# QuentinFuxa/WhisperLiveKit

Hardware: AMD Instinct MI355X
Metric: audio seconds transcribed per second (1/RTF), Whisper-base EN simul_whisper AlignAtt, 0.5 s chunks (higher is better)
Workload: dtype f32; 1 GPU; base.en simul_whisper, 1 stream(s) over 1 GPU(s) (1 per GPU), 30 s 16 kHz speech-like stream, 0.5 s chunks, beam 1, frame_threshold 25, seeded random weights, synthetic vocabulary; model=base.en, streams_total=1

## Files before the change

include/wlk_hip.h:

```cpp
#ifndef WLK_HIP_H
#define WLK_HIP_H

#include <stdint.h>

#ifdef __cplusplus
extern "C" {
#endif

#define WLK_OK 0
#define WLK_ERR_ARG (-1)
#define WLK_ERR_HIP (-2)
#define WLK_ERR_STATE (-3)
#define WLK_ERR_CAPACITY (-4)

typedef struct wlk_model wlk_model;
typedef struct wlk_session wlk_session;

typedef struct wlk_dims {
    int32_t n_mels, n_audio_ctx, n_audio_state, n_audio_head, n_audio_layer;
    int32_t n_vocab, n_text_ctx, n_text_state, n_text_head, n_text_layer;
} wlk_dims;

const char* wlk_last_error(void);
int wlk_abi_version(void);
// ... 159 lines not shown
int wlk_diag_env_refresh(void);
int wlk_diag_linear(const float* a, int64_t lda, int64_t a_floats, const float* w, const float* bias,
                    const float* r, int64_t ldr, int m, int n, int k, int flags, float scale, int scale_cols,
                    int force_gemv, float* c);
typedef struct wlk_nllb_dims {
    int32_t vocab, d_model, heads, ffn, enc_layers, dec_layers;
    int32_t max_src, max_tgt;
    int32_t pad_id;
    int32_t n_positions;
    float embed_scale;
} wlk_nllb_dims;
typedef struct wlk_nllb wlk_nllb;
typedef struct wlk_nllb_session wlk_nllb_session;
int wlk_nllb_arena_floats(const wlk_nllb_dims* dims, uint64_t* n_floats);
int wlk_nllb_tensor_lookup(const wlk_nllb_dims* dims, const char* packed_name, uint64_t* offset_floats, uint64_t* numel);
int wlk_nllb_tensor_name(const wlk_nllb_dims* dims, int index, const char** name);
int wlk_nllb_create(const wlk_nllb_dims* dims, int device, wlk_nllb** out);
int wlk_nllb_upload(wlk_nllb* m, const char* packed_name, const float* host, uint64_t numel);
int wlk_nllb_finalize(wlk_nllb* m);
int wlk_nllb_destroy(wlk_nllb* m);
int wlk_nllb_session_create(wlk_nllb* m, int rows, wlk_nllb_session** out);
int wlk_nllb_session_destroy(wlk_nllb_session* s);
int wlk_nllb_encode(wlk_nllb_session* s, const int64_t* src_ids, int32_t n);
int wlk_nllb_decode(wlk_nllb_session* s, const int64_t* tokens, int32_t n_rows, int32_t n_tok, int32_t first);
int wlk_nllb_step(wlk_nllb_session* s, const int64_t* tokens, int32_t n_rows, int32_t k, float* logprobs, int32_t* ids);
int wlk_nllb_kv_reorder(wlk_nllb_session* s, const int32_t* source_rows, int32_t n_rows);
int wlk_nllb_topk(wlk_nllb_session* s, int32_t k, float* logprobs, int32_t* ids);
int wlk_nllb_export(wlk_nllb_session* s, const char* what, float* host, uint64_t capacity, uint64_t* n_written);
int wlk_nllb_sync(wlk_nllb_session* s);

int wlk_dtw(int device, const float* x, int32_t n_rows, int32_t n_cols, int8_t* trace);
int wlk_log_mel(wlk_session* s, const float* pcm, int64_t n_samples, int32_t padding, float* mel, uint64_t capacity_floats,
                int32_t* n_frames);
int wlk_encode_mel(wlk_session* s, const float* mel, int32_t n_frames);
int wlk_find_alignment(wlk_session* s, const int64_t* tokens, int32_t n_tokens, int32_t n_sot, int32_t eot,
                       int32_t num_frames, float qk_scale, float* cost, int8_t* trace, float* token_probs);

int wlk_diag_linear_time(int m, int n, int k, int flags, int force_gemv, int reps, float* us_per_launch);
int wlk_diag_linear_ln(const float* a, const float* w, const float* bias, const float* gamma, const float* beta,
                       int m, int n, int k, int force_gemv, float* c);
int wlk_diag_layernorm(const float* x, const float* gamma, const float* beta, int rows, int d, float* y);
int wlk_diag_prefill_stack(wlk_session** sessions, const int64_t* tokens, const int32_t* n_tok, const int32_t* sot_index, int32_t n,
                           int32_t* taken);
int wlk_engine_prefill_stats(wlk_model* m, uint64_t* batches, uint64_t* sessions);
int wlk_diag_encoder_attention_time(int t, int d, int n_head, int k_splits, int reps, float* us_per_launch);
int wlk_diag_encoder_attention(const float* qkv, int t, int d, int n_head, float* out);
int wlk_diag_wave_ops(const float* in64, float* out640, float* ref640);
int wlk_diag_linear_x3(const float* a, const float* w, const float* bias, int m, int n, int k, int flags, float scale,
                       int scale_cols, float* c);
int wlk_diag_linear_x3_time(int m, int n, int k, int flags, int reps, float* us_per_launch);
int wlk_diag_layernorm_x3(const float* x, const float* gamma, const float* beta, int rows, int d, float* y);
int wlk_diag_encoder_attention_x3(const float* qkv, int t, int d, int n_head, float* out);
int wlk_diag_encoder_attention_x3_time(int t, int d, int n_head, int reps, float* us_per_launch);
int wlk_diag_qkv_x3_attention(const float* x, const float* w, const float* bias, int t, int d, int n_head, float scale,
                              float* out_epilogue, float* out_packed);

#ifdef __cplusplus
}
#endif
#endif
```

whisperlivekit_amd/_lib.py:

```python
from __future__ import annotations

import ctypes as C
import os
import threading
from typing import Optional


_LIB_NAME = "libwlk_hip.so"
_lock = threading.Lock()
_lib: Optional[C.CDLL] = None


class WlkError(RuntimeError):
    """Raised for every non-zero status of the C ABI (message from wlk_last_error())."""


class Dims(C.Structure):
    _fields_ = [(n, C.c_int32) for n in (
        "n_mels", "n_audio_ctx", "n_audio_state", "n_audio_head", "n_audio_layer",
        "n_vocab", "n_text_ctx", "n_text_state", "n_text_head", "n_text_layer")]


class SfDims(C.Structure):
    _fields_ = [(n, C.c_int32) for n in (
# ... 113 lines not shown
        "wlk_sf_finalize": (cint, [p]),
        "wlk_sf_step": (cint, [p, p, cint, p, cint, p, cint, C.POINTER(cint), p, cint]),
        "wlk_sf_step_pcm": (cint, [p, p, p, cint, cint, p, cint, p, cint, C.POINTER(cint), p, cint, p, cint, C.POINTER(cint), p, cint]),
        "wlk_sf_stats": (cint, [p, C.POINTER(u64), C.POINTER(u64), C.POINTER(u64)]),
        "wlk_sf_export": (cint, [p, C.c_char_p, p, u64, C.POINTER(u64)]),
        "wlk_sf_destroy": (cint, [p]),
        "wlk_nllb_arena_floats": (cint, [C.POINTER(NllbDims), C.POINTER(u64)]),
        "wlk_nllb_tensor_lookup": (cint, [C.POINTER(NllbDims), C.c_char_p, C.POINTER(u64), C.POINTER(u64)]),
        "wlk_nllb_tensor_name": (cint, [C.POINTER(NllbDims), cint, C.POINTER(C.c_char_p)]),
        "wlk_nllb_create": (cint, [C.POINTER(NllbDims), cint, C.POINTER(p)]),
        "wlk_nllb_upload": (cint, [p, C.c_char_p, p, u64]),
        "wlk_nllb_finalize": (cint, [p]),
        "wlk_nllb_destroy": (cint, [p]),
        "wlk_nllb_session_create": (cint, [p, cint, C.POINTER(p)]),
        "wlk_nllb_session_destroy": (cint, [p]),
        "wlk_nllb_encode": (cint, [p, p, i32]),
        "wlk_nllb_decode": (cint, [p, p, i32, i32, i32]),
        "wlk_nllb_step": (cint, [p, p, i32, i32, p, p]),
        "wlk_nllb_kv_reorder": (cint, [p, p, i32]),
        "wlk_nllb_topk": (cint, [p, i32, p, p]),
        "wlk_nllb_export": (cint, [p, C.c_char_p, p, u64, C.POINTER(u64)]),
        "wlk_nllb_sync": (cint, [p]),
        "wlk_vad_weights_floats": (cint, [C.POINTER(u64)]),
        "wlk_vad_tensor_lookup": (cint, [C.c_char_p, C.POINTER(u64), C.POINTER(u64)]),
        "wlk_vad_tensor_name": (cint, [cint, C.POINTER(C.c_char_p)]),
        "wlk_vad_create": (cint, [cint, p, u64, C.POINTER(p)]),
        "wlk_vad_destroy": (cint, [p]),
        "wlk_vad_stream_create": (cint, [p, cint, C.POINTER(p)]),
        "wlk_vad_stream_reset": (cint, [p]),
        "wlk_vad_stream_run": (cint, [p, p, cint, p]),
        "wlk_vad_stream_state": (cint, [p, p, p]),
        "wlk_vad_stream_destroy": (cint, [p]),
        "wlk_diag_last_error": (C.c_char_p, []),
        "wlk_diag_linear": (cint, [p, C.c_int64, C.c_int64, p, p, p, C.c_int64, cint, cint, cint, cint, C.c_float,
                                   cint, cint, p]),
        "wlk_dtw": (cint, [cint, C.POINTER(C.c_float), C.c_int32, C.c_int32, C.POINTER(C.c_int8)]),
        "wlk_encode_mel": (cint, [C.c_void_p, C.POINTER(C.c_float), C.c_int32]),
        "wlk_log_mel": (cint, [C.c_void_p, C.POINTER(C.c_float), C.c_int64, C.c_int32, C.POINTER(C.c_float), C.c_uint64,
                               C.POINTER(C.c_int32)]),
        "wlk_find_alignment": (cint, [C.c_void_p, C.POINTER(C.c_int64), C.c_int32, C.c_int32, C.c_int32, C.c_int32, C.c_float,
                                      C.POINTER(C.c_float), C.POINTER(C.c_int8), C.POINTER(C.c_float)]),
        "wlk_diag_linear_time": (cint, [cint, cint, cint, cint, cint, cint, C.POINTER(C.c_float)]),
        "wlk_diag_linear_ln": (cint, [p, p, p, p, p, cint, cint, cint, cint, p]),
        "wlk_diag_layernorm": (cint, [p, p, p, cint, cint, p]),
        "wlk_diag_encoder_attention_time": (cint, [cint, cint, cint, cint, cint, C.POINTER(C.c_float)]),
        "wlk_diag_encoder_attention": (cint, [p, cint, cint, cint, p]),
        "wlk_diag_wave_ops": (cint, [p, p, p]),
        "wlk_diag_env_refresh": (cint, []),
        "wlk_diag_linear_x3": (cint, [p, p, p, cint, cint, cint, cint, C.c_float, cint, p]),
        "wlk_diag_linear_x3_time": (cint, [cint, cint, cint, cint, cint, C.POINTER(C.c_float)]),
        "wlk_diag_layernorm_x3": (cint, [p, p, p, cint, cint, p]),
        "wlk_diag_encoder_attention_x3": (cint, [p, cint, cint, cint, p]),
        "wlk_diag_encoder_attention_x3_time": (cint, [cint, cint, cint, cint, C.POINTER(C.c_float)]),
        "wlk_diag_qkv_x3_attention": (cint, [p, p, p, cint, cint, cint, C.c_float, p, p]),
    }
    for name, (res, args) in sig.items():
        try:
            fn = getattr(lib, name)
        except AttributeError:
            if "WLK_HIP_LIB" in os.environ and name.startswith("wlk_diag_"):
                continue
            raise
        fn.restype = res
        fn.argtypes = args


EXPORTED_SYMBOLS = (
    "wlk_last_error", "wlk_abi_version", "wlk_device_count", "wlk_arena_floats", "wlk_tensor_lookup",
    "wlk_tensor_name", "wlk_model_create", "wlk_model_arena", "wlk_model_upload",
    "wlk_model_set_alignment_heads", "wlk_model_finalize", "wlk_model_destroy", "wlk_session_create",
    "wlk_session_destroy", "wlk_session_set_debug", "wlk_audio_append", "wlk_audio_append_pcm16", "wlk_audio_append_zeros",
    "wlk_audio_drop_front", "wlk_audio_clear", "wlk_audio_len", "wlk_encode", "wlk_decode",
    "wlk_no_speech_prob", "wlk_rules_set", "wlk_pick_greedy", "wlk_select", "wlk_kv_reorder", "wlk_sync", "wlk_decode_until_stop", "wlk_engine_attach", "wlk_engine_detach",
    "wlk_engine_stats", "wlk_engine_encode_stats", "wlk_engine_prefill_stats", "wlk_diag_prefill_stack", "wlk_job_create",
    "wlk_job_begin_step", "wlk_job_no_speech", "wlk_job_adjustments", "wlk_job_consume", "wlk_job_result",
    "wlk_job_destroy", "wlk_export", "wlk_session_step_stats", "wlk_prof_begin",
    "wlk_prof_end", "wlk_melspec_create", "wlk_melspec_run", "wlk_melspec_destroy",
    "wlk_sf_arena_floats", "wlk_sf_tensor_lookup", "wlk_sf_tensor_name", "wlk_sf_create", "wlk_sf_upload",
    "wlk_sf_finalize", "wlk_sf_step", "wlk_sf_step_pcm", "wlk_sf_stats", "wlk_sf_export", "wlk_sf_destroy",
    "wlk_vad_weights_floats", "wlk_vad_tensor_lookup", "wlk_vad_tensor_name", "wlk_vad_create", "wlk_vad_destroy",
    "wlk_vad_stream_create", "wlk_vad_stream_reset", "wlk_vad_stream_run", "wlk_vad_stream_state",
    "wlk_vad_stream_destroy",
    "wlk_dtw", "wlk_encode_mel", "wlk_log_mel", "wlk_find_alignment",
    "wlk_nllb_arena_floats", "wlk_nllb_tensor_lookup", "wlk_nllb_tensor_name", "wlk_nllb_create", "wlk_nllb_upload",
    "wlk_nllb_finalize", "wlk_nllb_destroy", "wlk_nllb_session_create", "wlk_nllb_session_destroy", "wlk_nllb_encode",
    "wlk_nllb_decode", "wlk_nllb_step", "wlk_nllb_kv_reorder", "wlk_nllb_topk", "wlk_nllb_export", "wlk_nllb_sync",
    "wlk_diag_last_error", "wlk_diag_linear", "wlk_diag_linear_time", "wlk_diag_linear_ln", "wlk_diag_layernorm",
    "wlk_diag_encoder_attention", "wlk_diag_encoder_attention_time", "wlk_diag_wave_ops", "wlk_diag_env_refresh",
    "wlk_diag_linear_x3", "wlk_diag_linear_x3_time", "wlk_diag_layernorm_x3",
    "wlk_diag_encoder_attention_x3", "wlk_diag_encoder_attention_x3_time", "wlk_diag_qkv_x3_attention",
)


def load() -> C.CDLL:
    global _lib
    if _lib is not None:
        return _lib
    with _lock:
        if _lib is None:
            path = lib_path()
            if not os.path.exists(path):
                raise WlkError(
                    f"{path} not found: build it with `python -m whisperlivekit_amd.build` "
                    "(hipcc, gfx950). There is no CPU fallback for the HIP backend.")
            try:
                import torch
            except Exception:
                pass
            try:
                lib = C.CDLL(path, mode=C.RTLD_GLOBAL)
            except OSError as e:
                raise WlkError(f"cannot load {path}: {e}") from e
            _declare(lib)
            _lib = lib
    return _lib


def check(rc: int) -> None:
    if rc != 0:
        msg = load().wlk_last_error()
        raise WlkError(f"wlk_hip error {rc}: {msg.decode('utf-8', 'replace') if msg else '?'}")


def device_count() -> int:
    return int(load().wlk_device_count())
```

whisperlivekit_amd/csrc/attention_x3.hip:

```cpp
#include <atomic>
#include <cstdlib>
#include <type_traits>

#include "common.h"
#include "wave_ops.h"
#include "x3.h"

namespace wlk {

namespace {
typedef float af32x4 __attribute__((ext_vector_type(4)));

constexpr int AX_QT = 64, AX_KT = 32;
constexpr int AX_K_ROW = 384;
constexpr int AX_V_ROW = 192;
constexpr int AX_K_BYTES = AX_KT * AX_K_ROW;
constexpr int AX_V_BYTES = 64 * AX_V_ROW;
constexpr int AX_TILE_BYTES = AX_K_BYTES + AX_V_BYTES;
constexpr int AX_SLOT_BYTES = 2 * AX_TILE_BYTES;
constexpr int AX_NB = 3, AX_DT = AX_NB - 1;
constexpr int AX_NPW = AX_SLOT_BYTES / 1024 / 8;
constexpr size_t AX_LDS_BYTES = (size_t)AX_NB * AX_SLOT_BYTES;
constexpr int AX_PA[6] = {2, 0, 1, 1, 0, 0}, AX_PB[6] = {0, 2, 1, 0, 1, 0};

template <int N, int I = 0, typename F>
__device__ __forceinline__ void ax_static_for(F&& f) {
    if constexpr (I < N) {
        f(std::integral_constant<int, I>{});
        ax_static_for<N, I + 1>(f);
    }
}
__device__ __forceinline__ void ax_read12(af32x4 (&f)[12], const unsigned (&addr)[12], unsigned off) {
#pragma unroll
    for (int t = 0; t < 12; ++t) asm volatile("ds_read_b128 %0, %1" : "=v"(f[t]) : "v"(addr[t] + off));
}
__device__ __forceinline__ void ax_wait12(af32x4 (&f)[12]) {
    asm volatile("s_waitcnt lgkmcnt(0)" : "+v"(f[0]), "+v"(f[1]), "+v"(f[2]), "+v"(f[3]), "+v"(f[4]), "+v"(f[5]));
    asm volatile("" : "+v"(f[6]), "+v"(f[7]), "+v"(f[8]), "+v"(f[9]), "+v"(f[10]), "+v"(f[11]));
}
__device__ __forceinline__ void ax_split8(const float (&v)[8], bf16x8 (&out)[3]) {
#pragma unroll
    for (int e = 0; e < 8; ++e) {
        const X3Triple t = x3_split(v[e]);
        out[0][e] = t.h;
        out[1][e] = t.m;
        out[2][e] = t.l;
    }
}
__host__ __device__ inline int ax_vt_key(int u, int e) { return 4 * u + (e & 3) + 16 * (e >> 2); }
}

struct AttnX3Args {
    const unsigned short* qk3;
    long ldqk;
// ... 183 lines not shown
    }
    asm volatile("s_waitcnt vmcnt(0)" ::: "memory");
    __builtin_amdgcn_s_barrier();

    constexpr int O_LD = 68;
    float* Os = reinterpret_cast<float*>(lds);
    float* Ms = Os + 8 * 16 * O_LD;
    float* Ls = Ms + 8 * 16;
#pragma unroll
    for (int db = 0; db < 4; ++db)
#pragma unroll
        for (int i = 0; i < 4; ++i) Os[(wave * 16 + c) * O_LD + 16 * db + 4 * g + i] = o[db][i];
    if (g == 0) {
        Ms[wave * 16 + c] = m_run;
        Ls[wave * 16 + c] = l_run;
    }
    asm volatile("s_waitcnt lgkmcnt(0)" ::: "memory");
    __builtin_amdgcn_s_barrier();
    if (a.x3_out) {
        const int tid = threadIdx.x;
        const int q = tid >> 3, ch = tid & 7;
        const int qrow = q0 + q;
        const int w0 = q >> 4, w1 = w0 + 4;
        const float m0 = Ms[w0 * 16 + (q & 15)], m1 = Ms[w1 * 16 + (q & 15)];
        const float M = fmaxf(m0, m1);
        const float e0 = m0 == -INFINITY ? 0.f : expf(m0 - M), e1 = m1 == -INFINITY ? 0.f : expf(m1 - M);
        const float L = e0 * Ls[w0 * 16 + (q & 15)] + e1 * Ls[w1 * 16 + (q & 15)];
        float v[8];
#pragma unroll
        for (int e = 0; e < 8; ++e) {
            const int dd = 8 * ch + e;
            v[e] = (e0 * Os[(w0 * 16 + (q & 15)) * O_LD + dd] + e1 * Os[(w1 * 16 + (q & 15)) * O_LD + dd]) / L;
        }
        if (qrow < T)
            x3_store_chunk(reinterpret_cast<unsigned short*>(aout) + (long)qrow * 3 * a.ldo + (long)(head * 8 + ch) * 24, v);
    } else {
        const int tid = threadIdx.x;
        const int dd = tid & 63, qg = tid >> 6;
#pragma unroll
        for (int i = 0; i < 8; ++i) {
            const int q = qg * 8 + i;
            const int qrow = q0 + q;
            const int w0 = q >> 4, w1 = w0 + 4;
            const float m0 = Ms[w0 * 16 + (q & 15)], m1 = Ms[w1 * 16 + (q & 15)];
            const float M = fmaxf(m0, m1);
            const float e0 = m0 == -INFINITY ? 0.f : expf(m0 - M), e1 = m1 == -INFINITY ? 0.f : expf(m1 - M);
            const float L = e0 * Ls[w0 * 16 + (q & 15)] + e1 * Ls[w1 * 16 + (q & 15)];
            const float acc = e0 * Os[(w0 * 16 + (q & 15)) * O_LD + dd] + e1 * Os[(w1 * 16 + (q & 15)) * O_LD + dd];
            if (qrow < T) aout[(long)qrow * a.ldo + head * 64 + dd] = acc / L;
        }
    }
}

__global__ __launch_bounds__(256) void x3_pack_qkv_kernel(const float* __restrict__ qkv, unsigned short* __restrict__ out, int T, int d,
                                                          long vt_off, long vt_ld) {
    const long n_qk = (long)T * (2 * d / 8), n_vt = (long)d * (vt_ld / 8);
    const long idx = (long)blockIdx.x * 256 + threadIdx.x;
    float v[8];
    if (idx < n_qk) {
        const int row = (int)(idx / (2 * d / 8)), c = (int)(idx - (long)row * (2 * d / 8));
#pragma unroll
        for (int e = 0; e < 8; ++e) v[e] = qkv[(long)row * 3 * d + 8 * c + e];
        x3_store_chunk(out + (long)row * 3 * (2 * d) + (long)c * 24, v);
    } else if (idx < n_qk + n_vt) {
        const long j = idx - n_qk;
        const int dcol = (int)(j / (vt_ld / 8)), u = (int)(j - (long)dcol * (vt_ld / 8));
#pragma unroll
        for (int e = 0; e < 8; ++e) {
            const int t = 32 * (u >> 2) + ax_vt_key(u & 3, e);
            v[e] = t < T ? qkv[(long)t * 3 * d + 2 * d + dcol] : 0.f;
        }
        x3_store_chunk(out + vt_off + (long)dcol * 3 * vt_ld + (long)u * 24, v);
    }
}

void launch_x3_pack_qkv(const LaunchCtx& ctx, const float* qkv, unsigned short* out, int T, int d, long vt_off, long vt_ld) {
    const long n = (long)T * (2 * d / 8) + (long)d * (vt_ld / 8);
    KernelScope ks(ctx, "x3_pack_qkv");
    hipLaunchKernelGGL(x3_pack_qkv_kernel, dim3((unsigned)((n + 255) / 256)), dim3(256), 0, ctx.stream, qkv, out, T, d, vt_off, vt_ld);
    WLK_HIP(hipGetLastError());
}

bool enc_attention_x3_enabled() {
    static const bool on = [] {
        const char* e = getenv("WLK_X3_ATTN");
        return !(e && e[0] == '0');
    }();
    return on;
}

void launch_encoder_attention_x3(const LaunchCtx& ctx, const unsigned short* qk3, long ldqk, long vt_off, long vt_ld, float* out,
                                 long ldo, int T, int d, int n_head, const PtrTable* z, int batch, bool x3_out) {
    if (d != n_head * 64 || ldqk % 8 != 0 || vt_ld % 32 != 0 || vt_ld < ((T + 31) / 32) * 32 || T < 64)
        throw std::invalid_argument("x3 attention: unsupported shape");
    static std::atomic<uint64_t> configured{0};
    int dev = 0;
    WLK_HIP(hipGetDevice(&dev));
    if (!(configured.load(std::memory_order_acquire) >> (dev & 63) & 1)) {
        WLK_HIP(hipFuncSetAttribute(reinterpret_cast<const void*>(&enc_attention_x3_kernel<0>), hipFuncAttributeMaxDynamicSharedMemorySize, (int)AX_LDS_BYTES));
        WLK_HIP(hipFuncSetAttribute(reinterpret_cast<const void*>(&enc_attention_x3_kernel<1>), hipFuncAttributeMaxDynamicSharedMemorySize, (int)AX_LDS_BYTES));
        WLK_HIP(hipFuncSetAttribute(reinterpret_cast<const void*>(&enc_attention_x3_kernel<2>), hipFuncAttributeMaxDynamicSharedMemorySize, (int)AX_LDS_BYTES));
        WLK_HIP(hipFuncSetAttribute(reinterpret_cast<const void*>(&enc_attention_x3_kernel<3>), hipFuncAttributeMaxDynamicSharedMemorySize, (int)AX_LDS_BYTES));
        configured.fetch_or(1ull << (dev & 63), std::memory_order_release);
    }
    AttnX3Args a{};
    a.qk3 = qk3; a.ldqk = ldqk; a.vt_off = vt_off; a.vt_ld = vt_ld; a.out = out; a.ldo = ldo; a.T = T; a.d = d; a.n_head = n_head;
    a.batch = batch;
    a.x3_out = x3_out ? 1 : 0;
    if (x3_out && ldo % 8 != 0) throw std::invalid_argument("x3 attention: X3 result rows need ldo % 8 == 0");
    if (batch > 0) a.z = *z;
    const int q_tiles = (T + AX_QT - 1) / AX_QT;
    KernelScope ks(ctx, "enc_attention_x3", (batch > 0 ? batch : 1) * 4.0 * (double)T * T * 64 * n_head, 0.0);
    static const int abl = [] {
        const char* e = getenv("WLK_X3_ATTN_ABL");
        return e ? atoi(e) : 0;
    }();
    const dim3 grid(q_tiles * n_head, batch > 0 ? batch : 1);
    if (abl == 1) hipLaunchKernelGGL(enc_attention_x3_kernel<1>, grid, dim3(512), AX_LDS_BYTES, ctx.stream, a);
    else if (abl == 2) hipLaunchKernelGGL(enc_attention_x3_kernel<2>, grid, dim3(512), AX_LDS_BYTES, ctx.stream, a);
    else if (abl == 3) hipLaunchKernelGGL(enc_attention_x3_kernel<3>, grid, dim3(512), AX_LDS_BYTES, ctx.stream, a);
    else hipLaunchKernelGGL(enc_attention_x3_kernel<0>, grid, dim3(512), AX_LDS_BYTES, ctx.stream, a);
    WLK_HIP(hipGetLastError());
}

}
```

whisperlivekit_amd/csrc/diag.hip:

```cpp
#include <cstdio>
#include <cstdlib>
#include <vector>

#include "../../include/wlk_hip.h"
#include "common.h"
#include "internal.h"
#include "wave_ops.h"

using namespace wlk;

namespace {
thread_local std::string g_diag_error;
struct DevBuf {
    float* p = nullptr;
    explicit DevBuf(size_t n, const float* host = nullptr) {
        WLK_HIP(hipMalloc(reinterpret_cast<void**>(&p), std::max<size_t>(n, 1) * sizeof(float)));
        if (host) WLK_HIP(hipMemcpy(p, host, n * sizeof(float), hipMemcpyHostToDevice));
    }
    ~DevBuf() { (void)hipFree(p); }
};
template <typename F>
int run(F&& f) {
    try {
        f();
// ... 328 lines not shown
        launch_x3_pack_w(ctx, W.p, k, w3, n, k);
        X3GemmArgs g;
        g.A3 = a3; g.lda = k; g.W3 = w3; g.bias = B.p; g.C = Cc.p; g.ldc = n; g.M = m; g.N = n; g.K = k; g.flags = flags;
        g.scale = 0.5f; g.scale_cols = n / 2;
        launch_gemm_x3(ctx, g, "diag");
        WLK_HIP(hipStreamSynchronize(st));
        hipEvent_t e0, e1;
        WLK_HIP(hipEventCreate(&e0));
        WLK_HIP(hipEventCreate(&e1));
        WLK_HIP(hipEventRecord(e0, st));
        for (int i = 0; i < reps; ++i) launch_gemm_x3(ctx, g, "diag");
        WLK_HIP(hipEventRecord(e1, st));
        WLK_HIP(hipStreamSynchronize(st));
        float ms = 0.f;
        WLK_HIP(hipEventElapsedTime(&ms, e0, e1));
        *us_per_launch = 1e3f * ms / (float)reps;
        (void)hipEventDestroy(e0);
        (void)hipEventDestroy(e1);
        (void)hipStreamDestroy(st);
        (void)hipFree(a3);
        (void)hipFree(w3);
    });
}

int wlk_diag_layernorm_x3(const float* x, const float* gamma, const float* beta, int rows, int d, float* y) {
    return run([&]() {
        DevBuf X((size_t)rows * d, x), G(d, gamma), Bt(d, beta), Y((size_t)rows * d);
        unsigned short* y3 = nullptr;
        WLK_HIP(hipMalloc(reinterpret_cast<void**>(&y3), (size_t)rows * 3 * d * sizeof(unsigned short)));
        LaunchCtx ctx;
        launch_layernorm_x3(ctx, X.p, d, G.p, Bt.p, y3, d, rows, d, "diag_ln_x3");
        launch_x3_unpack(ctx, y3, d, Y.p, d, rows, d);
        WLK_HIP(hipDeviceSynchronize());
        WLK_HIP(hipMemcpy(y, Y.p, (size_t)rows * d * sizeof(float), hipMemcpyDeviceToHost));
        (void)hipFree(y3);
    });
}

int wlk_diag_encoder_attention_x3(const float* qkv, int t, int d, int n_head, float* out) {
    return run([&]() {
        DevBuf Q((size_t)t * 3 * d, qkv), O((size_t)t * d);
        unsigned short* img = nullptr;
        const size_t n = x3_attn_image_elems(t, d);
        WLK_HIP(hipMalloc(reinterpret_cast<void**>(&img), n * sizeof(unsigned short)));
        LaunchCtx ctx;
        launch_x3_pack_qkv(ctx, Q.p, img, t, d, x3_attn_vt_off(t, d), x3_attn_vt_ld(t));
        launch_encoder_attention_x3(ctx, img, 2L * d, x3_attn_vt_off(t, d), x3_attn_vt_ld(t), O.p, d, t, d, n_head, nullptr, 0);
        WLK_HIP(hipDeviceSynchronize());
        WLK_HIP(hipMemcpy(out, O.p, (size_t)t * d * sizeof(float), hipMemcpyDeviceToHost));
        (void)hipFree(img);
    });
}

int wlk_diag_qkv_x3_attention(const float* x, const float* w, const float* bias, int t, int d, int n_head, float scale,
                              float* out_epilogue, float* out_packed) {
    return run([&]() {
        DevBuf X((size_t)t * d, x), W((size_t)3 * d * d, w), B((size_t)3 * d, bias), QKV((size_t)t * 3 * d), O((size_t)t * d);
        unsigned short *x3 = nullptr, *w3 = nullptr, *img = nullptr;
        const size_t n_img = x3_attn_image_elems(t, d);
        WLK_HIP(hipMalloc(reinterpret_cast<void**>(&x3), (size_t)t * 3 * d * sizeof(unsigned short)));
        WLK_HIP(hipMalloc(reinterpret_cast<void**>(&w3), x3_w_elems(3 * d, d) * sizeof(unsigned short)));
        WLK_HIP(hipMalloc(reinterpret_cast<void**>(&img), n_img * sizeof(unsigned short)));
        LaunchCtx ctx;
        launch_x3_pack(ctx, X.p, d, x3, d, t, d);
        launch_x3_pack_w(ctx, W.p, d, w3, 3 * d, d);
        X3GemmArgs g;
        g.A3 = x3; g.lda = d; g.W3 = w3; g.bias = B.p; g.M = t; g.N = 3 * d; g.K = d;
        g.flags = kGemmScaleCols; g.scale = scale; g.scale_cols = 2 * d;
        for (int route = 0; route < 2; ++route) {
            WLK_HIP(hipMemset(img, 0, n_img * sizeof(unsigned short)));
            X3GemmArgs r = g;
            if (route == 0) {
                r.x3_out = true; r.C3 = img; r.ldc3 = 2 * d; r.vt_col0 = 2 * d; r.vt_off = x3_attn_vt_off(t, d); r.vt_ld = x3_attn_vt_ld(t);
                launch_gemm_x3(ctx, r, "diag_qkv_x3");
            } else {
                r.C = QKV.p; r.ldc = 3 * d;
                launch_gemm_x3(ctx, r, "diag_qkv");
                launch_x3_pack_qkv(ctx, QKV.p, img, t, d, x3_attn_vt_off(t, d), x3_attn_vt_ld(t));
            }
            launch_encoder_attention_x3(ctx, img, 2L * d, x3_attn_vt_off(t, d), x3_attn_vt_ld(t), O.p, d, t, d, n_head, nullptr, 0);
            WLK_HIP(hipDeviceSynchronize());
            WLK_HIP(hipMemcpy(route == 0 ? out_epilogue : out_packed, O.p, (size_t)t * d * sizeof(float), hipMemcpyDeviceToHost));
        }
        (void)hipFree(x3);
        (void)hipFree(w3);
        (void)hipFree(img);
    });
}

int wlk_diag_encoder_attention_x3_time(int t, int d, int n_head, int reps, float* us_per_launch) {
    return run([&]() {
        std::vector<float> h((size_t)t * 3 * d);
        unsigned seed = 777u;
        for (auto& v : h) { seed = seed * 1664525u + 1013904223u; v = (((seed >> 8) & 0xffff) / 65536.0f - 0.5f) * 1.5f; }
        DevBuf Q((size_t)t * 3 * d, h.data()), O((size_t)t * d);
        unsigned short* img = nullptr;
        WLK_HIP(hipMalloc(reinterpret_cast<void**>(&img), x3_attn_image_elems(t, d) * sizeof(unsigned short)));
        hipStream_t st;
        WLK_HIP(hipStreamCreateWithFlags(&st, hipStreamNonBlocking));
        LaunchCtx ctx{st, nullptr};
        launch_x3_pack_qkv(ctx, Q.p, img, t, d, x3_attn_vt_off(t, d), x3_attn_vt_ld(t));
        auto go = [&]() { launch_encoder_attention_x3(ctx, img, 2L * d, x3_attn_vt_off(t, d), x3_attn_vt_ld(t), O.p, d, t, d, n_head, nullptr, 0); };
        go();
        WLK_HIP(hipStreamSynchronize(st));
        hipEvent_t e0, e1;
        WLK_HIP(hipEventCreate(&e0));
// ... 17 lines not shown
```

whisperlivekit_amd/csrc/gemm_f32.hip:

```cpp
#include <algorithm>
#include <atomic>
#include <cstdio>
#include <cstdlib>
#include <type_traits>

#include "common.h"
#include "wave_ops.h"
#include "align_body.h"

namespace wlk {

typedef float f32x16 __attribute__((ext_vector_type(16)));
typedef float f32x4 __attribute__((ext_vector_type(4)));
typedef unsigned int u32x4 __attribute__((ext_vector_type(4)));

constexpr int BK = 32, LDS_LD = BK + 4;

__device__ __forceinline__ float gelu_erf(float x) {
    return 0.5f * x * (1.0f + erff(x * 0.70710678118654752440f));
}

template <int NA, int NW>
struct Stage {
    float4 a[NA], w[NW];
// ... 967 lines not shown
    using Cfg = KSplitCfg<TM, TN, KS>;
    static_assert(Cfg::LDS_BYTES <= 160 * 1024, "tile does not fit the 160 KiB LDS");
    static std::atomic<uint64_t> configured{0};
    int dev = 0;
    WLK_HIP(hipGetDevice(&dev));
    if (!(configured.load(std::memory_order_acquire) >> (dev & 63) & 1)) {
        WLK_HIP(hipFuncSetAttribute(reinterpret_cast<const void*>(&gemm_nt_f32_ksplit_kernel<TM, TN, KS, ABL>),
                                    hipFuncAttributeMaxDynamicSharedMemorySize, (int)Cfg::LDS_BYTES));
        configured.fetch_or(1ull << (dev & 63), std::memory_order_release);
    }
    const int tiles_m = (g.M + Cfg::BM - 1) / Cfg::BM, tiles_n = (g.N + Cfg::BN - 1) / Cfg::BN;
    const int blocks = tiles_m >= 8 ? 8 * ((tiles_m + 3) / 4) * ((tiles_n + 1) / 2) : tiles_m * tiles_n;
    hipLaunchKernelGGL((gemm_nt_f32_ksplit_kernel<TM, TN, KS, ABL>), dim3(blocks, std::max(g.batch, 1)), dim3(256), Cfg::LDS_BYTES,
                       ctx.stream, g);
}

template <int KS, int ABL>
static bool dispatch_ksplit(const LaunchCtx& ctx, const GemmArgs& g, int tm, int tn) {
#define WLK_KS(a, b) if (tm == a && tn == b) { launch_ksplit<a, b, KS, ABL>(ctx, g); return true; }
    WLK_KS(3, 4) WLK_KS(3, 3) WLK_KS(3, 2) WLK_KS(3, 1) WLK_KS(2, 4) WLK_KS(2, 2) WLK_KS(2, 1) WLK_KS(4, 2)
#undef WLK_KS
    return false;
}

static long kwave_max_tiles() {
    static const long v = [] {
        const char* e = getenv("WLK_KWAVE_MAX_TILES");
        return e ? atol(e) : 416L;
    }();
    return v;
}

bool gemm_takes_kwave(int M, int N, int K) {
    const long tiles32 = (long)((N + 31) / 32) * ((M + 31) / 32);
    return K >= 256 && tiles32 <= kwave_max_tiles();
}

bool gemm_takes_ksplit(int M, int N, int K) { return ksplit_tile(M, N, K).tm != 0; }

static bool kwave16_enabled() {
    static const bool on = [] {
        const char* e = getenv("WLK_KWAVE16");
        return !(e && e[0] == '0');
    }();
    return on;
}

static bool gemm_can_fuse_layernorm(int M, int N, int K) {
    return kwave16_enabled() && M > 8 && M <= 128 && gemm_takes_kwave(M, N, K) && ksplit_tile(M, N, K).tm == 0 &&
           (K == 384 || K == 512 || K == 768 || K == 1024 || K == 1280);
}
static std::atomic<int> g_prefill_ln_fuse{-1};
void x3_refresh_env_switches();
void refresh_env_switches() {
    g_prefill_ln_fuse.store(-1, std::memory_order_relaxed);
    x3_refresh_env_switches();
}
bool gemm_fuses_layernorm(int M, int N, int K) {
    int on = g_prefill_ln_fuse.load(std::memory_order_relaxed);
    if (on < 0) {
        const char* e = getenv("WLK_PREFILL_LN_FUSE");
        on = e && e[0] == '1';
        g_prefill_ln_fuse.store(on, std::memory_order_relaxed);
    }
    return on && gemm_can_fuse_layernorm(M, N, K);
}

void launch_gemm(const LaunchCtx& ctx, const GemmArgs& g, const char* tag) {
    if (g.M <= 0 || g.N <= 0) return;
    if (g.K % 4 != 0 || g.lda % 4 != 0) throw std::invalid_argument("gemm: K and lda must be multiples of 4");
    if ((((long)g.M - 1) * g.lda + g.K) * 4 >= (1L << 31) || (long)g.N * g.K * 4 >= (1L << 31))
        throw std::invalid_argument("gemm: operand larger than 2 GiB");
    const double nb = std::max(g.batch, 1);
    KernelScope ks(ctx, tag, nb * 2.0 * g.M * g.N * g.K,
                   4.0 * (nb * (double)g.M * g.K + (double)g.N * g.K + nb * (double)g.M * g.N));
    if (g.batch > kMaxBatch) throw std::invalid_argument("gemm: batch too large");
    const bool want_kwave = g.force_kwave || g.force_kernel == 2;
    const KSplitTile kt = (want_kwave || g.kcache || g.force_kernel == 3) ? KSplitTile{0, 0, 0} : ksplit_tile(g.M, g.N, g.K, g.force_kernel == 4);
    if (g.force_kernel == 4 && !kt.tm) throw std::invalid_argument("gemm: the k-split kernel does not take this shape");
    if (g.ln_gamma && !(gemm_can_fuse_layernorm(g.M, g.N, g.K) && !kt.tm && g.force_kernel == 0 && g.batch == 0))
        throw std::invalid_argument("gemm: only the 16 x 16 prefill kernel takes the LayerNorm (gemm_fuses_layernorm)");
    if (kt.tm) {
        static const KSplitTile forced = [] {
            KSplitTile f{0, 0, 0};
            if (const char* e = getenv("WLK_KSPLIT_FORCE")) sscanf(e, "%d,%d,%d", &f.tm, &f.tn, &f.ks);
            return f;
        }();
        const KSplitTile use = forced.tm ? forced : kt;
        bool ok;
        if (use.ks >= 100) ok = dispatch_kpipe(ctx, g, use.tm, use.tn, use.ks);
        else ok = dispatch_ksplit<64, 0>(ctx, g, use.tm, use.tn);
        if (!ok) throw std::logic_error("gemm: k-split tile without an instantiation");
        WLK_HIP(hipGetLastError());
        return;
    }
    if (g.batch > 0 && (gemm_takes_kwave(g.M, g.N, g.K) || want_kwave || (long)((g.N + 63) / 64) * ((g.M + 63) / 64) < 64))
        throw std::invalid_argument("gemm: batched launches are only available on the tiled paths");
    const long tiles64 = (long)((g.N + 63) / 64) * ((g.M + 63) / 64);
    const int tiles_n = (g.N + 63) / 64;
    const long tiles32 = (long)((g.N + 31) / 32) * ((g.M + 31) / 32);
    if (g.kcache && !(gemm_takes_kwave(g.M, g.N, g.K) || want_kwave))
        throw std::invalid_argument("gemm: fused KV-cache append is only available on the k-wave path");
    if ((gemm_takes_kwave(g.M, g.N, g.K) && g.force_kernel != 3) || (want_kwave && g.K >= 256)) {
        if (kwave16_enabled() && g.M <= 128 && g.force_kernel != 2) {
            const long tiles16 = (long)((g.N + 15) / 16) * ((g.M + 15) / 16);
            const dim3 grid((unsigned)tiles16);
            switch (g.ln_gamma ? g.K / 64 : 0) {
                case 0: hipLaunchKernelGGL(gemm_nt_f32_kwave16_kernel<0>, grid, dim3(256), 0, ctx.stream, g); break;
                case 6: hipLaunchKernelGGL(gemm_nt_f32_kwave16_kernel<6>, grid, dim3(256), 0, ctx.stream, g); break;
// ... 690 lines not shown
```

Before: 208.2 audio_s/s.

## Add key-split balanced encoder attention kernel with CU-aware auto selection

Adds an alternative x3 encoder attention kernel in which each workgroup runs 12 waves: 3 query sub-tiles each split across 4 key partitions. Partial softmax states are merged through LDS at the end. A heuristic based on CU count, tile count and workgroup count picks this kernel over the existing one when its estimated per-CU work is lower, which targets poor CU occupancy at small T and batch. The cost is an extra LDS reduction and a larger block, and it can be overridden with an environment variable.

Result: faster. 212.3 audio_s/s (median of 6 runs) (+2.0%).

```diff
diff --git a/include/wlk_hip.h b/include/wlk_hip.h
--- a/include/wlk_hip.h
+++ b/include/wlk_hip.h
@@ -235,6 +235,7 @@
 int wlk_diag_layernorm_x3(const float* x, const float* gamma, const float* beta, int rows, int d, float* y);
 int wlk_diag_encoder_attention_x3(const float* qkv, int t, int d, int n_head, float* out);
 int wlk_diag_encoder_attention_x3_time(int t, int d, int n_head, int reps, float* us_per_launch);
+int wlk_diag_encoder_attention_x3_batch(const float* qkv, int batch, int t, int d, int n_head, int x3_out, float* out);
 int wlk_diag_qkv_x3_attention(const float* x, const float* w, const float* bias, int t, int d, int n_head, float scale,
                               float* out_epilogue, float* out_packed);
 
diff --git a/whisperlivekit_amd/_lib.py b/whisperlivekit_amd/_lib.py
--- a/whisperlivekit_amd/_lib.py
+++ b/whisperlivekit_amd/_lib.py
@@ -189,6 +189,7 @@
         "wlk_diag_layernorm_x3": (cint, [p, p, p, cint, cint, p]),
         "wlk_diag_encoder_attention_x3": (cint, [p, cint, cint, cint, p]),
         "wlk_diag_encoder_attention_x3_time": (cint, [cint, cint, cint, cint, C.POINTER(C.c_float)]),
+        "wlk_diag_encoder_attention_x3_batch": (cint, [p, cint, cint, cint, cint, cint, p]),
         "wlk_diag_qkv_x3_attention": (cint, [p, p, p, cint, cint, cint, C.c_float, p, p]),
     }
     for name, (res, args) in sig.items():
@@ -226,6 +227,7 @@
     "wlk_diag_encoder_attention", "wlk_diag_encoder_attention_time", "wlk_diag_wave_ops", "wlk_diag_env_refresh",
     "wlk_diag_linear_x3", "wlk_diag_linear_x3_time", "wlk_diag_layernorm_x3",
     "wlk_diag_encoder_attention_x3", "wlk_diag_encoder_attention_x3_time", "wlk_diag_qkv_x3_attention",
+    "wlk_diag_encoder_attention_x3_batch",
 )
 
 
diff --git a/whisperlivekit_amd/csrc/attention_x3.hip b/whisperlivekit_amd/csrc/attention_x3.hip
--- a/whisperlivekit_amd/csrc/attention_x3.hip
+++ b/whisperlivekit_amd/csrc/attention_x3.hip
@@ -1,5 +1,7 @@
+#include <algorithm>
 #include <atomic>
 #include <cstdlib>
+#include <cstring>
 #include <type_traits>
 
 #include "common.h"
@@ -289,6 +291,214 @@
     }
 }
 
+constexpr int AB_QB = 3, AB_KS = 4, AB_WAVES = AB_QB * AB_KS, AB_QT = 16 * AB_QB;
+constexpr size_t AB_LDS_BYTES = (size_t)AB_KS * AX_TILE_BYTES;
+
+template <int OFF>
+__device__ __forceinline__ void ab_read(af32x4& f, unsigned addr) {
+    asm volatile("ds_read_b128 %0, %1 offset:%2" : "=v"(f) : "v"(addr), "i"(OFF));
+}
+
+__global__ __launch_bounds__(AB_WAVES * 64) void enc_attention_x3_bal_kernel(AttnX3Args a) {
+    asm volatile("" ::"s"(a.qk3), "s"(a.ldqk), "s"(a.vt_off), "s"(a.vt_ld), "s"(a.out), "s"(a.ldo), "s"(a.T), "s"(a.d), "s"(a.n_head),
+                 "s"(a.batch));
+    __builtin_amdgcn_sched_barrier(0);
+    extern __shared__ __attribute__((aligned(1024))) unsigned char lds[];
+    const int lane = threadIdx.x & 63;
+    const int wave = __builtin_amdgcn_readfirstlane(threadIdx.x >> 6);
+    const bool batched = a.batch > 0;
+    const unsigned short* const qk3 = batched ? reinterpret_cast<const unsigned short*>(table_at(a.z.in, blockIdx.y)) : a.qk3;
+    float* const aout = batched ? table_at(a.z.out, blockIdx.y) : a.out;
+    const int T = a.T;
+    const int head = blockIdx.x % a.n_head;
+    const int q0 = (blockIdx.x / a.n_head) * AB_QT;
+    const int n_tiles = (T + AX_KT - 1) / AX_KT;
+    const int n_steps = (n_tiles + AB_KS - 1) / AB_KS;
+    const long row_qk = 3 * a.ldqk * 2, row_vt = 3 * a.vt_ld * 2;
+    const int qs = wave % AB_QB, ks = wave / AB_QB;
+    const int c = lane & 15, g = lane >> 4;
+    const bool live = q0 + 16 * qs < T;
+
+    bf16x8 qf[6];
+    {
+        const int q = min(q0 + 16 * qs + c, T - 1);
+        const char* qp = reinterpret_cast<const char*>(qk3) + (long)q * row_qk + (long)(head * 8) * 48;
+#pragma unroll
+        for (int kstep = 0; kstep < 2; ++kstep)
+#pragma unroll
+            for (int p = 0; p < 3; ++p)
+                qf[kstep * 3 + p] = __builtin_bit_cast(bf16x8, *reinterpret_cast<const x3_u32x4*>(qp + ((4 * kstep + g) * 3 + p) * 16));
+    }
+    const int pb = 1024 * wave + 16 * lane;
+    const int k_row = pb / AX_K_ROW;
+    const int k_up = (pb - k_row * AX_K_ROW) >> 4;
+    const char* const img = reinterpret_cast<const char*>(qk3);
+    const unsigned k_off = (unsigned)((a.d / 8 + head * 8) * 48 + (((k_up / 3) ^ (k_row & 7)) * 3 + k_up % 3) * 16);
+    const int v_row = pb / AX_V_ROW;
+    const int v_up = (pb - v_row * AX_V_ROW) >> 4;
+    const unsigned v_off = (unsigned)(a.vt_off * 2 + (long)(head * 64 + v_row) * row_vt + (((v_up / 3) ^ ((v_row >> 1) & 3)) * 3 + v_up % 3) * 16);
+    auto issue_step = [&](int step) {
+        ax_static_for<AB_KS>([&](auto S) {
+            constexpr int s = decltype(S)::value;
+            const int tile = AB_KS * step + s;
+            const int key = min(tile * AX_KT + k_row, T - 1);
+            const int vt = min(tile, n_tiles - 1);
+            __builtin_amdgcn_global_load_lds((const __attribute__((address_space(1))) void*)(img + (k_off + (unsigned)key * (unsigned)row_qk)),
+                                             (__attribute__((address_space(3))) void*)(lds + s * AX_TILE_BYTES + wave * 1024), 16, 0, 0);
+            __builtin_amdgcn_global_load_lds((const __attribute__((address_space(1))) void*)(img + (v_off + (unsigned)vt * ((AX_KT / 8) * 48))),
+                                             (__attribute__((address_space(3))) void*)(lds + s * AX_TILE_BYTES + AX_K_BYTES + wave * 1024),
+                                             16, 0, 0);
+        });
+    };
+    issue_step(0);
+
+    const unsigned tile_base = (unsigned)(size_t)(__attribute__((address_space(3))) unsigned char*)lds + (unsigned)ks * AX_TILE_BYTES;
+    const unsigned k_base0 = tile_base + (unsigned)(c * AX_K_ROW) + (unsigned)((((0 + g) ^ (c & 7)) * 3) * 16);
+    const unsigned k_base1 = tile_base + (unsigned)(c * AX_K_ROW) + (unsigned)((((4 + g) ^ (c & 7)) * 3) * 16);
+    const unsigned v_base = tile_base + AX_K_BYTES + (unsigned)(c * AX_V_ROW) + (unsigned)(((g ^ ((c >> 1) & 3)) * 3) * 16);
+    af32x4 o[4];
+#pragma unroll
+    for (int db = 0; db < 4; ++db) o[db] = af32x4{0.f, 0.f, 0.f, 0.f};
+    float m_run = -INFINITY, l_run = 0.f;
+
+    asm volatile("s_waitcnt vmcnt(0)" ::: "memory");
+    __builtin_amdgcn_s_barrier();
+    for (int st = 0; st < n_steps; ++st) {
+        const int tile = AB_KS * st + ks;
+        const bool act = live && tile < n_tiles;
+        af32x4 s2[2] = {af32x4{0.f, 0.f, 0.f, 0.f}, af32x4{0.f, 0.f, 0.f, 0.f}};
+        af32x4 vf[12];
+        if (act) {
+            af32x4 kf[12];
+            ax_static_for<12>([&](auto X) {
+                constexpr int x = decltype(X)::value;
+                constexpr int kb = x / 6, kstep = (x / 3) % 2, p = x % 3;
+                ab_read<kb * 16 * AX_K_ROW + p * 16>(kf[x], kstep ? k_base1 : k_base0);
+            });
+            ax_wait12(kf);
+            ax_static_for<24>([&](auto X) {
+                constexpr int x = decltype(X)::value;
+                constexpr int t = x / 4, kstep = (x / 2) % 2, kb = x % 2;
+                s2[kb] = __builtin_amdgcn_mfma_f32_16x16x32_bf16(__builtin_bit_cast(bf16x8, kf[kb * 6 + kstep * 3 + AX_PA[t]]),
+                                                                 qf[kstep * 3 + AX_PB[t]], s2[kb], 0, 0, 0);
+            });
+            __builtin_amdgcn_sched_barrier(0);
+            ax_static_for<12>([&](auto X) {
+                constexpr int x = decltype(X)::value;
+                ab_read<(x / 3) * 16 * AX_V_ROW + (x % 3) * 16>(vf[x], v_base);
+            });
+            ax_wait12(vf);
+        }
+        __builtin_amdgcn_s_barrier();
+        if (st + 1 < n_steps) issue_step(st + 1);
+        if (act) {
+            float s[8];
+#pragma unroll
+            for (int i = 0; i < 4; ++i) { s[i] = s2[0][i]; s[4 + i] = s2[1][i]; }
+            const int key0 = tile * AX_KT;
+            if (__builtin_amdgcn_readfirstlane(key0 + AX_KT > T)) {
+#pragma unroll
+                for (int i = 0; i < 8; ++i)
+                    if (key0 + 16 * (i >> 2) + 4 * g + (i & 3) >= T) s[i] = -INFINITY;
+            }
+            float mt = fmaxf(fmaxf(fmaxf(s[0], s[1]), fmaxf(s[2], s[3])), fmaxf(fmaxf(s[4], s[5]), fmaxf(s[6], s[7])));
+            mt = fmaxf(mt, wave_xor<16>(mt));
+            mt = fmaxf(mt, wave_xor<32>(mt));
+            const float m_new = fmaxf(m_run, mt);
+            const float alpha = __expf(m_run - m_new);
+            float rs = 0.f;
+#pragma unroll
+            for (int i = 0; i < 8; ++i) {
+                s[i] = __expf(s[i] - m_new);
+                rs += s[i];
+            }
+            rs += wave_xor<16>(rs);
+            rs += wave_xor<32>(rs);
+            l_run = l_run * alpha + rs;
+            m_run = m_new;
+            if (__builtin_amdgcn_ballot_w64(alpha != 1.0f) != 0) {
+#pragma unroll
+                for (int db = 0; db < 4; ++db) o[db] *= alpha;
+            }
+            bf16x8 pf[3];
+            ax_split8(s, pf);
+            ax_static_for<24>([&](auto X) {
+                constexpr int x = decltype(X)::value;
+                constexpr int t = x / 4, db = x % 4;
+                o[db] = __builtin_amdgcn_mfma_f32_16x16x32_bf16(__builtin_bit_cast(bf16x8, vf[db * 3 + AX_PA[t]]), pf[AX_PB[t]], o[db], 0, 0, 0);
+            });
+        }
+        asm volatile("s_waitcnt vmcnt(0)" ::: "memory");
+        __builtin_amdgcn_s_barrier();
+    }
+
+    constexpr int O_LD = 68;
+    float* Os = reinterpret_cast<float*>(lds);
+    float* Ms = Os + AB_WAVES * 16 * O_LD;
+    float* Ls = Ms + AB_WAVES * 16;
+#pragma unroll
+    for (int db = 0; db < 4; ++db)
+#pragma unroll
+        for (int i = 0; i < 4; ++i) Os[(wave * 16 + c) * O_LD + 16 * db + 4 * g + i] = o[db][i];
+    if (g == 0) {
+        Ms[wave * 16 + c] = m_run;
+        Ls[wave * 16 + c] = l_run;
+    }
+    asm volatile("s_waitcnt lgkmcnt(0)" ::: "memory");
+    __builtin_amdgcn_s_barrier();
+    auto weights = [&](int q, float (&e)[AB_KS], int (&r)[AB_KS]) {
+        float m[AB_KS], M = -INFINITY;
+#pragma unroll
+        for (int k = 0; k < AB_KS; ++k) {
+            r[k] = ((q >> 4) + AB_QB * k) * 16 + (q & 15);
+            m[k] = Ms[r[k]];
+            M = fmaxf(M, m[k]);
+        }
+        float L = 0.f;
+#pragma unroll
+        for (int k = 0; k < AB_KS; ++k) {
+            e[k] = m[k] == -INFINITY ? 0.f : expf(m[k] - M);
+            L += e[k] * Ls[r[k]];
+        }
+        return L;
+    };
+    const int tid = threadIdx.x;
+    if (a.x3_out) {
+        const int q = tid >> 3, ch = tid & 7;
+        const int qrow = q0 + q;
+        if (q < AB_QT && qrow < T) {
+            float e[AB_KS];
+            int r[AB_KS];
+            const float L = weights(q, e, r);
+            float v[8];
+#pragma unroll
+            for (int j = 0; j < 8; ++j) {
+                float acc = 0.f;
+#pragma unroll
+                for (int k = 0; k < AB_KS; ++k) acc += e[k] * Os[r[k] * O_LD + 8 * ch + j];
+                v[j] = acc / L;
+            }
+            x3_store_chunk(reinterpret_cast<unsigned short*>(aout) + (long)qrow * 3 * a.ldo + (long)(head * 8 + ch) * 24, v);
+        }
+    } else {
+        const int dd = tid & 63, qg = tid >> 6;
+#pragma unroll
+        for (int i = 0; i < 4; ++i) {
+            const int q = qg * 4 + i;
+            const int qrow = q0 + q;
+            if (qrow < T) {
+                float e[AB_KS];
+                int r[AB_KS];
+                const float L = weights(q, e, r);
+                float acc = 0.f;
+#pragma unroll
+                for (int k = 0; k < AB_KS; ++k) acc += e[k] * Os[r[k] * O_LD + dd];
+                aout[(long)qrow * a.ldo + head * 64 + dd] = acc / L;
+            }
+        }
+    }
+}
+
 __global__ __launch_bounds__(256) void x3_pack_qkv_kernel(const float* __restrict__ qkv, unsigned short* __restrict__ out, int T, int d,
                                                           long vt_off, long vt_ld) {
     const long n_qk = (long)T * (2 * d / 8), n_vt = (long)d * (vt_ld / 8);
@@ -324,6 +534,38 @@
         return !(e && e[0] == '0');
     }();
     return on;
+}
+
+static std::atomic<int> g_x3_attn_form{-1};
+void x3_attention_refresh_env_switches() { g_x3_attn_form.store(-1, std::memory_order_relaxed); }
+static int x3_attn_form() {
+    int f = g_x3_attn_form.load(std::memory_order_relaxed);
+    if (f < 0) {
+        const char* e = getenv("WLK_X3_ATTN_FORM");
+        f = !e ? 0 : !strcmp(e, "r4") ? 1 : !strcmp(e, "bal") ? 2 : 0;
+        g_x3_attn_form.store(f, std::memory_order_relaxed);
+    }
+    return f;
+}
+static int device_cus() {
+    static std::atomic<int> cus[64];
+    int dev = 0;
+    WLK_HIP(hipGetDevice(&dev));
+    int n = cus[dev & 63].load(std::memory_order_relaxed);
+    if (n <= 0) {
+        WLK_HIP(hipDeviceGetAttribute(&n, hipDeviceAttributeMultiprocessorCount, dev));
+        cus[dev & 63].store(n, std::memory_order_relaxed);
+    }
+    return n;
+}
+static bool x3_attn_balanced(int T, int n_head, int nb) {
+    const int form = x3_attn_form();
+    if (form) return form == 2;
+    const long cus = device_cus(), n_tiles = (T + AX_KT - 1) / AX_KT;
+    const long wg_r4 = (long)(T + AX_QT - 1) / AX_QT * n_head * nb, wg_bal = (long)(T + AB_QT - 1) / AB_QT * n_head * nb;
+    const long r4 = (wg_r4 + cus - 1) / cus * 2 * ((n_tiles + 1) / 2);
+    const long bal = (wg_bal + cus - 1) / cus * AB_QB * ((n_tiles + AB_KS - 1) / AB_KS);
+    return bal < r4;
 }
 
 void launch_encoder_attention_x3(const LaunchCtx& ctx, const unsigned short* qk3, long ldqk, long vt_off, long vt_ld, float* out,
@@ -338,6 +580,7 @@
         WLK_HIP(hipFuncSetAttribute(reinterpret_cast<const void*>(&enc_attention_x3_kernel<1>), hipFuncAttributeMaxDynamicSharedMemorySize, (int)AX_LDS_BYTES));
         WLK_HIP(hipFuncSetAttribute(reinterpret_cast<const void*>(&enc_attention_x3_kernel<2>), hipFuncAttributeMaxDynamicSharedMemorySize, (int)AX_LDS_BYTES));
         WLK_HIP(hipFuncSetAttribute(reinterpret_cast<const void*>(&enc_attention_x3_kernel<3>), hipFuncAttributeMaxDynamicSharedMemorySize, (int)AX_LDS_BYTES));
+        WLK_HIP(hipFuncSetAttribute(reinterpret_cast<const void*>(&enc_attention_x3_bal_kernel), hipFuncAttributeMaxDynamicSharedMemorySize, (int)AB_LDS_BYTES));
         configured.fetch_or(1ull << (dev & 63), std::memory_order_release);
     }
     AttnX3Args a{};
@@ -346,13 +589,21 @@
     a.x3_out = x3_out ? 1 : 0;
     if (x3_out && ldo % 8 != 0) throw std::invalid_argument("x3 attention: X3 result rows need ldo % 8 == 0");
     if (batch > 0) a.z = *z;
-    const int q_tiles = (T + AX_QT - 1) / AX_QT;
-    KernelScope ks(ctx, "enc_attention_x3", (batch > 0 ? batch : 1) * 4.0 * (double)T * T * 64 * n_head, 0.0);
+    const int nb = batch > 0 ? batch : 1;
+    KernelScope ks(ctx, "enc_attention_x3", nb * 4.0 * (double)T * T * 64 * n_head, 0.0);
     static const int abl = [] {
         const char* e = getenv("WLK_X3_ATTN_ABL");
         return e ? atoi(e) : 0;
     }();
-    const dim3 grid(q_tiles * n_head, batch > 0 ? batch : 1);
+    if (abl == 0 && x3_attn_balanced(T, n_head, nb)) {
+        if (std::max((long)T * 3 * ldqk, vt_off + (long)d * 3 * vt_ld) * 2 >= (1L << 31))
+            throw std::invalid_argument("x3 attention: operand image larger than 2 GiB");
+        const dim3 grid((T + AB_QT - 1) / AB_QT * n_head, nb);
+        hipLaunchKernelGGL(enc_attention_x3_bal_kernel, grid, dim3(AB_WAVES * 64), AB_LDS_BYTES, ctx.stream, a);
+        WLK_HIP(hipGetLastError());
+        return;
+    }
+    const dim3 grid((T + AX_QT - 1) / AX_QT * n_head, nb);
     if (abl == 1) hipLaunchKernelGGL(enc_attention_x3_kernel<1>, grid, dim3(512), AX_LDS_BYTES, ctx.stream, a);
     else if (abl == 2) hipLaunchKernelGGL(enc_attention_x3_kernel<2>, grid, dim3(512), AX_LDS_BYTES, ctx.stream, a);
     else if (abl == 3) hipLaunchKernelGGL(enc_attention_x3_kernel<3>, grid, dim3(512), AX_LDS_BYTES, ctx.stream, a);
diff --git a/whisperlivekit_amd/csrc/diag.hip b/whisperlivekit_amd/csrc/diag.hip
--- a/whisperlivekit_amd/csrc/diag.hip
+++ b/whisperlivekit_amd/csrc/diag.hip
@@ -404,6 +404,30 @@
     });
 }
 
+int wlk_diag_encoder_attention_x3_batch(const float* qkv, int batch, int t, int d, int n_head, int x3_out, float* out) {
+    return run([&]() {
+        if (batch < 1 || batch > kMaxBatch) throw std::invalid_argument("diag: batch out of range");
+        if (d % 64 != 0) throw std::invalid_argument("diag: d must be a multiple of 64");
+        DevBuf Q((size_t)batch * t * 3 * d, qkv), O((size_t)batch * t * d);
+        const size_t n = x3_attn_image_elems(t, d);
+        DevBuf img_buf((size_t)batch * n / 2), o3_buf(x3_out ? (size_t)batch * t * 3 * d / 2 : 0);
+        unsigned short* const img = reinterpret_cast<unsigned short*>(img_buf.p);
+        unsigned short* const o3 = reinterpret_cast<unsigned short*>(o3_buf.p);
+        LaunchCtx ctx;
+        PtrTable z{};
+        for (int i = 0; i < batch; ++i) {
+            launch_x3_pack_qkv(ctx, Q.p + (size_t)i * t * 3 * d, img + (size_t)i * n, t, d, x3_attn_vt_off(t, d), x3_attn_vt_ld(t));
+            z.in[i] = reinterpret_cast<const float*>(img + (size_t)i * n);
+            z.out[i] = x3_out ? reinterpret_cast<float*>(o3 + (size_t)i * t * 3 * d) : O.p + (size_t)i * t * d;
+        }
+        launch_encoder_attention_x3(ctx, nullptr, 2L * d, x3_attn_vt_off(t, d), x3_attn_vt_ld(t), nullptr, d, t, d, n_head, &z, batch, x3_out != 0);
+        if (x3_out)
+            for (int i = 0; i < batch; ++i) launch_x3_unpack(ctx, o3 + (size_t)i * t * 3 * d, d, O.p + (size_t)i * t * d, d, t, d);
+        WLK_HIP(hipDeviceSynchronize());
+        WLK_HIP(hipMemcpy(out, O.p, (size_t)batch * t * d * sizeof(float), hipMemcpyDeviceToHost));
+    });
+}
+
 int wlk_diag_qkv_x3_attention(const float* x, const float* w, const float* bias, int t, int d, int n_head, float scale,
                               float* out_epilogue, float* out_packed) {
     return run([&]() {
diff --git a/whisperlivekit_amd/csrc/gemm_f32.hip b/whisperlivekit_amd/csrc/gemm_f32.hip
--- a/whisperlivekit_amd/csrc/gemm_f32.hip
+++ b/whisperlivekit_amd/csrc/gemm_f32.hip
@@ -1043,9 +1043,11 @@
 }
 static std::atomic<int> g_prefill_ln_fuse{-1};
 void x3_refresh_env_switches();
+void x3_attention_refresh_env_switches();
 void refresh_env_switches() {
     g_prefill_ln_fuse.store(-1, std::memory_order_relaxed);
     x3_refresh_env_switches();
+    x3_attention_refresh_env_switches();
 }
 bool gemm_fuses_layernorm(int M, int N, int K) {
     int on = g_prefill_ln_fuse.load(std::memory_order_relaxed);
```
